# rubengooj/pl-svo

Measured on NVIDIA H100. Metric: frame-pair aligns/sec (VGA 5-lvl pyr, ~300pt+80ln), higher is better.
Workload: dtype f32 residuals, weights and chi2 (the reference's summation order, bit-exact); f64 per-pixel normal equations, solve and SE3

## Files before the change

### pl-svo_b200/csrc/align_kernel.cu

```cuda
#include <cuda_runtime.h>
#include <stdint.h>

#include "device_math.cuh"
#include "internal.h"

namespace plsvo {

namespace {

#ifdef PLSVO_PHASE_CLOCKS
enum {
  kPhSetup, kPhPtEval, kPhPtChi2, kPhSeg, kPhReduce,
  kPhSerRed, kPhSerSolve, kPhSerWalk, kPhSerSegSum, kPhSerBar1, kPhSerDecide, kPhSerFinal,
  kPhPair, kNumPhases
};
__device__ unsigned long long g_phase_clocks[kNumPhases];
#define PHASE_MARK(k)                        \
  do {                                       \
    const int ptid_ = fresh_tid();           \
    if ((ptid_ & 31) == 0) {                 \
      const long long now_ = clock64();      \
      ph_acc[ptid_ >> 5][k] += now_ - ph_t[ptid_ >> 5]; \
      ph_t[ptid_ >> 5] = now_;               \
    }                                        \
  } while (0)
#else
#define PHASE_MARK(k) \
  do {                \
  } while (0)
#endif

struct PairCtl {
  double R[9];
  double t[3];
  double model[7];
  double old_model[7];
  double T_ref[7];
  double ref_pos[3];
  double chi2_prev;
  double H_last[36];
  double scratch[36];
  double g[6];
  double x[6];
  unsigned long long mbar;
  long long n_meas_last;
  int pair;
  int flag;
  int stop;
  int iter;
  int n_seg_patches;
  int n_seg_slots;
  unsigned int patch_iters;
  unsigned int patch_levels;
  int iters_level[PLSVO_MAX_LEVELS];
  double cand[7];
  double candR[9];
  double cand_nm;
  double dscale, cJ, cJ2;
  float seg_chi2f;
  float chi2f;
  int n_opq;
  int chi2_flags;
};

struct Layout {
  uint32_t ctl, red, tot, chunk_tot, items, cnt, flat, opq, seg_N0, seg_N, seg_off, seg_slot, slot_seg, seg_term,
      seg_alive, pt_vis, xyz, tsc, img, total;
};

__host__ __device__ inline uint32_t align_up(uint32_t v, uint32_t a) { return (v + a - 1) / a * a; }

__host__ __device__ inline Layout make_layout(int n_pts, int n_segs, int max_patches, int max_seg_slots, int img_bytes,
                                              int nt) {
  Layout L;
  const uint32_t nw = (uint32_t)nt / 32u;
  const uint32_t rounds = ((uint32_t)n_pts + (uint32_t)nt - 1u) / (uint32_t)nt;
  const uint32_t n_chunks = ((uint32_t)n_pts + 31u) / 32u;
  uint32_t o = 0;
  L.ctl = o;
  o = align_up(o + (uint32_t)sizeof(PairCtl), 16);
  L.red = o;
  o += nw * 32u * 8u;
  L.tot = o;
  o += 32u * 8u;
  L.chunk_tot = o;
  o += 8u * (rounds * nw + 1u);
  L.items = o;
  o += 8u * 32u * (n_chunks + 1u);
  L.cnt = o;
  o += 4u * (n_chunks + 1u);
  L.flat = align_up(o, 8);
  o = L.flat + 8u * 64u;
  L.seg_N0 = o;
  o += 4u * (uint32_t)n_segs;
  L.seg_N = o;
  o += 4u * (uint32_t)n_segs;
  L.seg_off = o;
  o += 4u * (uint32_t)n_segs;
  L.seg_slot = o;
  o += 4u * (uint32_t)n_segs;
  L.slot_seg = o;
  o += 2u * (uint32_t)max_seg_slots;
  L.seg_term = align_up(o, 4);
  o = L.seg_term;
  o += 4u * (uint32_t)n_segs;
  L.seg_alive = o;
  o += (uint32_t)n_segs;
  L.pt_vis = o;
  o += (uint32_t)n_pts;
  L.xyz = align_up(o, 16);
  o = L.xyz + 3u * 8u * (uint32_t)max_patches;
  L.tsc = o;
  o += 16u * 4u * (uint32_t)nt;
  o = align_up(o, 128);
  L.img = o;
  o += (uint32_t)img_bytes + 16u;
  L.opq = align_up(o, 16);
  o = L.opq + 64u * (uint32_t)align_opq_cap(n_pts);
  L.total = o;
  return L;
}

__device__ __forceinline__ float bilin(float wTL, float wTR, float wBL, float wBR, float a, float b, float c, float d) {
  return __fadd_rn(__fadd_rn(__fadd_rn(__fmul_rn(wTL, a), __fmul_rn(wTR, b)), __fmul_rn(wBL, c)), __fmul_rn(wBR, d));
}

__device__ __forceinline__ bool patch_setup(double u, double v, int cols, int rows, int boundary, int& ui, int& vi,
                                            float& wTL, float& wTR, float& wBL, float& wBR) {
  const float uf = (float)u, vf = (float)v;
  const float fu = floorf(uf), fv = floorf(vf);
  ui = (int)fu;
  vi = (int)fv;
  if (ui < boundary || vi < boundary || ui >= cols - boundary || vi >= rows - boundary) return false;
  const float su = __fsub_rn(uf, fu), sv = __fsub_rn(vf, fv);
  const float omu = __fsub_rn(1.0f, su), omv = __fsub_rn(1.0f, sv);
  wTL = __fmul_rn(omu, omv);
  wTR = __fmul_rn(su, omv);
  wBL = __fmul_rn(omu, sv);
  wBR = __fmul_rn(su, sv);
  return true;
}

__device__ __noinline__ int seg_num_samples0(const double* spx, const double* epx, double length) {
  const double a0 = fabs(epx[0] - spx[0]), a1 = fabs(epx[1] - spx[1]);
  const double tan_dir = __ddiv_rn(fmin(a0, a1), fmax(a0, a1));
  const double sin_dir = __ddiv_rn(tan_dir, __dsqrt_rn(__dadd_rn(1.0, __dmul_rn(tan_dir, tan_dir))));
  const double correction = __dmul_rn(2.0, __dsqrt_rn(__dadd_rn(1.0, __dmul_rn(sin_dir, sin_dir))));
  double nd = __ddiv_rn(length, __dmul_rn(8.0, correction));
  if (!(nd >= 1.0)) nd = 1.0;
  if (nd > 1048576.0) nd = 1048576.0;
  return (int)(unsigned long long)nd;
}

__device__ __forceinline__ bool cam_in_frame(int ox, int oy, int boundary, int level, int width, int height) {
  return ox >= boundary && ox < width / (1 << level) - boundary && oy >= boundary &&
         oy < height / (1 << level) - boundary;
}

__device__ __forceinline__ void cam2world(const AlignArgs& a, const double* px, double* f) {
  const double x = __ddiv_rn(__dsub_rn(px[0], a.cx), a.fx), y = __ddiv_rn(__dsub_rn(px[1], a.cy), a.fy);
  const double n = __dsqrt_rn(__dadd_rn(__dadd_rn(__dmul_rn(x, x), __dmul_rn(y, y)), 1.0));
  f[0] = __ddiv_rn(x, n), f[1] = __ddiv_rn(y, n), f[2] = __ddiv_rn(1.0, n);
}

__device__ __forceinline__ void rank2_update(double* acc, double xn, double yn, double zi, double Sxx, double Sxy,
                                             double Syy, double Sxr, double Syr) {
  double r0[6], r1[6];
  const double xy = xn * yn;
  r0[0] = -zi, r0[1] = 0.0, r0[2] = xn * zi, r0[3] = xy, r0[4] = -(1.0 + xn * xn), r0[5] = yn;
  r1[0] = 0.0, r1[1] = -zi, r1[2] = yn * zi, r1[3] = 1.0 + yn * yn, r1[4] = -xy, r1[5] = -xn;
  double p[6], q[6];
#pragma unroll
  for (int i = 0; i < 6; ++i) {
    p[i] = Sxx * r0[i] + Sxy * r1[i];
    q[i] = Sxy * r0[i] + Syy * r1[i];
  }
  int idx = 0;
#pragma unroll
  for (int i = 0; i < 6; ++i)
#pragma unroll
    for (int j = i; j < 6; ++j) acc[idx++] += p[i] * r0[j] + q[i] * r1[j];
#pragma unroll
  for (int i = 0; i < 6; ++i) acc[21 + i] -= Sxr * r0[i] + Syr * r1[i];
}

__device__ __forceinline__ void load_row5(const uint8_t* row, int sh, uint32_t& lo, uint32_t& hi) {
  const uint32_t w0 = *reinterpret_cast<const uint32_t*>(row);
  const uint32_t w1 = *reinterpret_cast<const uint32_t*>(row + 4);
  lo = __funnelshift_r(w0, w1, sh);
  hi = w1 >> sh;
}
__device__ __forceinline__ float row_px(uint32_t lo, uint32_t hi, int k) {
  return k < 4 ? byte_to_float(lo, k) : byte_to_float(hi, 0);
}

__device__ __forceinline__ void project(const PairCtl* ctl, const AlignArgs& a, double xn, double yn, double zi, double& u,
                                        double& v) {
  const double* R = ctl->R;
  const double* t = ctl->t;
  const double xc = R[0] * xn + R[1] * yn + (R[2] + t[0] * zi);
  const double yc = R[3] * xn + R[4] * yn + (R[5] + t[1] * zi);
  const double zc = R[6] * xn + R[7] * yn + (R[8] + t[2] * zi);
  const double izc = __drcp_rn(zc);
  u = (a.fx * (xc * izc) + a.cx) * ctl->dscale;
  v = (a.fy * (yc * izc) + a.cy) * ctl->dscale;
}
__device__ __forceinline__ void load_row7(const uint8_t* row, int sh, float* g) {
  const uint32_t* wp = reinterpret_cast<const uint32_t*>(row);
  const uint32_t w0 = __ldg(wp), w1 = __ldg(wp + 1), w2 = __ldg(wp + 2);
  const uint32_t lo = __funnelshift_r(w0, w1, sh);
  const uint32_t hi = __funnelshift_r(w1, w2, sh);
  g[0] = byte_to_float(lo, 0);
  g[1] = byte_to_float(lo, 1);
  g[2] = byte_to_float(lo, 2);
  g[3] = byte_to_float(lo, 3);
  g[4] = byte_to_float(hi, 0);
  g[5] = byte_to_float(hi, 1);
  g[6] = byte_to_float(hi, 2);
}

template <bool weighted, int NT>
__device__ __forceinline__ bool eval_patch(const uint8_t* __restrict__ img, int pitch, int cols, int rows,
                                           const float4* __restrict__ cache, int MP, int p, double u, double v,
                                           double* S , float* __restrict__ tsc, float& tsum) {
  int ui, vi;
  float wTL, wTR, wBL, wBR;
  if (!patch_setup(u, v, cols, rows, 2, ui, vi, wTL, wTR, wBL, wBR)) return false;
  const int c0 = ui - 2;
  const int sh = (c0 & 3) * 8;
  const uint8_t* rowp = img + (size_t)(vi - 2) * pitch + (c0 & ~3);
  uint32_t ra_lo, ra_hi, rb_lo, rb_hi;
  load_row5(rowp, sh, ra_lo, ra_hi);
#ifdef PLSVO_FP32_SUMS
  float Sxx = 0.f, Sxy = 0.f, Syy = 0.f, Sxr = 0.f, Syr = 0.f;
#else
  double Sxx = 0, Sxy = 0, Syy = 0, Sxr = 0, Syr = 0;
#endif
  float acc_f = 0.f;
  const float4* cp = cache + p;
#pragma unroll 1
  for (int y = 0; y < 4; ++y) {
    rowp += pitch;
    load_row5(rowp, sh, rb_lo, rb_hi);
    const float4 ref4 = cp[0];
    const float4 dx4 = cp[4 * MP];
    const float4 dy4 = cp[8 * MP];
    cp += MP;
    const float refv[4] = {ref4.x, ref4.y, ref4.z, ref4.w};
    const float dxv[4] = {dx4.x, dx4.y, dx4.z, dx4.w};
    const float dyv[4] = {dy4.x, dy4.y, dy4.z, dy4.w};
#pragma unroll
    for (int x = 0; x < 4; ++x) {
      const float cur = bilin(wTL, wTR, wBL, wBR, row_px(ra_lo, ra_hi, x), row_px(ra_lo, ra_hi, x + 1),
                              row_px(rb_lo, rb_hi, x), row_px(rb_lo, rb_hi, x + 1));
      const float res = __fsub_rn(cur, refv[x]);
      const float dx = dxv[x], dy = dyv[x];
      const float ares = fabsf(res);
      const float nw = weighted ? -weight_rcp(ares) : -1.0f;
      const float nterm = weighted ? __fmul_rn(__fmul_rn(res, res), nw) : -ares;
      tsc[(y * 4 + x) * NT] = nterm;
      acc_f = __fsub_rn(acc_f, nterm);
#ifdef PLSVO_FP32_SUMS
      const float wdx = weighted ? __fmul_rn(-nw, dx) : dx, wdy = weighted ? __fmul_rn(-nw, dy) : dy;
      Sxx = fmaf(wdx, dx, Sxx);
      Sxy = fmaf(wdx, dy, Sxy);
      Syy = fmaf(wdy, dy, Syy);
      Sxr = fmaf(wdx, res, Sxr);
      Syr = fmaf(wdy, res, Syr);
#else
      const double dxd = (double)dx, dyd = (double)dy, rd = (double)res;
      const double nwdx = weighted ? (double)nw * dxd : -dxd;
      const double nwdy = weighted ? (double)nw * dyd : -dyd;
      Sxx = fma(-nwdx, dxd, Sxx);
      Sxy = fma(-nwdx, dyd, Sxy);
      Syy = fma(-nwdy, dyd, Syy);
      Sxr = fma(-nwdx, rd, Sxr);
      Syr = fma(-nwdy, rd, Syr);
#endif
    }
    ra_lo = rb_lo, ra_hi = rb_hi;
  }
  S[0] = (double)Sxx, S[1] = (double)Sxy, S[2] = (double)Syy, S[3] = (double)Sxr, S[4] = (double)Syr;
  tsum = acc_f;
  return true;
}

template <int NT>
__device__ __forceinline__ float chain16(float s, const float* tsc) {
#pragma unroll
  for (int k = 0; k < 16; ++k) s = __fsub_rn(s, tsc[k * NT]);
  return s;
}
template <int NT>
__device__ __forceinline__ void chain16x2(float& s0, float& s1, const float* tsc) {
#pragma unroll
  for (int k = 0; k < 16; ++k) {
    const float t = tsc[k * NT];
    s0 = __fsub_rn(s0, t);
    s1 = __fsub_rn(s1, t);
  }
}

__device__ __forceinline__ void precompute_patch(const uint8_t* __restrict__ img, int pitch, int ui, int vi, float wTL,
                                                 float wTR, float wBL, float wBR, float4* __restrict__ cache, int MP,
                                                 int p) {
  const int c0 = ui - 3;
  const int sh = (c0 & 3) * 8;
  const uint8_t* rowp = img + (size_t)(vi - 3) * pitch + (c0 & ~3);
  float g0[7], g1[7], Va[6], Vb[6], Vc[6];
  load_row7(rowp, sh, g0);
  load_row7(rowp + pitch, sh, g1);
#pragma unroll
  for (int c = 0; c < 6; ++c) Va[c] = bilin(wTL, wTR, wBL, wBR, g0[c], g0[c + 1], g1[c], g1[c + 1]);
  rowp += 2 * pitch;
  load_row7(rowp, sh, g0);
#pragma unroll
  for (int c = 0; c < 6; ++c) Vb[c] = bilin(wTL, wTR, wBL, wBR, g1[c], g1[c + 1], g0[c], g0[c + 1]);
  float4* cp = cache + p;
#pragma unroll 1
  for (int y = 0; y < 4; ++y) {
    rowp += pitch;
    load_row7(rowp, sh, g1);
#pragma unroll
    for (int c = 0; c < 6; ++c) Vc[c] = bilin(wTL, wTR, wBL, wBR, g0[c], g0[c + 1], g1[c], g1[c + 1]);
    float refv[4], dxv[4], dyv[4];
#pragma unroll
    for (int x = 0; x < 4; ++x) {
      refv[x] = Vb[x + 1];
      dxv[x] = __fmul_rn(0.5f, __fsub_rn(Vb[x + 2], Vb[x]));
      dyv[x] = __fmul_rn(0.5f, __fsub_rn(Vc[x + 1], Va[x + 1]));
    }
    cp[0] = make_float4(refv[0], refv[1], refv[2], refv[3]);
    cp[4 * MP] = make_float4(dxv[0], dxv[1], dxv[2], dxv[3]);
    cp[8 * MP] = make_float4(dyv[0], dyv[1], dyv[2], dyv[3]);
    cp += MP;
#pragma unroll
    for (int c = 0; c < 6; ++c) Va[c] = Vb[c], Vb[c] = Vc[c];
#pragma unroll
    for (int c = 0; c < 7; ++c) g0[c] = g1[c];
  }
}

__device__ __forceinline__ void zero_gradients(float4* cache, int MP, int p) {
  const float4 z = make_float4(0.f, 0.f, 0.f, 0.f);
#pragma unroll
  for (int y = 0; y < 8; ++y) cache[(4 + y) * MP + p] = z;
}

__device__ __noinline__ void gn_solve(PairCtl* ctl, const double* tot, int level) {
  ctl->n_meas_last = (long long)tot[28];
  ctl->patch_iters += (unsigned int)tot[29];
  ctl->iters_level[level] += 1;
  double xx[6];
  {
    double Hu[21], gg[6];
#pragma unroll
    for (int i = 0; i < 21; ++i) Hu[i] = tot[i];
#pragma unroll
    for (int i = 0; i < 6; ++i) gg[i] = tot[21 + i];
    if (!ldlt6_reg(Hu, gg, xx)) {
      double* H = ctl->H_last;
      int idx = 0;
      for (int i = 0; i < 6; ++i)
        for (int j = i; j < 6; ++j) {
          H[i * 6 + j] = tot[idx];
          H[j * 6 + i] = tot[idx];
          ++idx;
        }
      for (int i = 0; i < 6; ++i) ctl->g[i] = tot[21 + i];
      ldlt6_solve(H, ctl->g, ctl->x, ctl->scratch);
#pragma unroll
      for (int i = 0; i < 6; ++i) xx[i] = ctl->x[i];
    }
  }
  if (isnan(xx[0])) ctl->stop = 1;
  double mx[6];
  double nm = 0.0;
#pragma unroll
  for (int i = 0; i < 6; ++i) {
    mx[i] = -xx[i];
    nm = fmax(nm, fabs(xx[i]));
  }
  SE3q model;
  model.q.x = ctl->model[0], model.q.y = ctl->model[1], model.q.z = ctl->model[2], model.q.w = ctl->model[3];
  model.t = v3(ctl->model[4], ctl->model[5], ctl->model[6]);
  const SE3q cand = se3_mul(model, se3_exp(mx));
  se3_store(cand, ctl->cand);
  quat_to_R(cand.q, ctl->candR);
  ctl->cand_nm = nm;
}

__device__ __noinline__ void gn_decide(PairCtl* ctl, const double* tot, float chi2f, int n_iter, double eps) {
  const double new_chi2 = (double)(chi2f / (float)(unsigned long long)ctl->n_meas_last);
  const bool reject = (ctl->iter > 0 && new_chi2 > ctl->chi2_prev) || ctl->stop;
  int flag;
  if (reject) {
    for (int i = 0; i < 7; ++i) ctl->model[i] = ctl->old_model[i];
    Quat q;
    q.x = ctl->model[0], q.y = ctl->model[1], q.z = ctl->model[2], q.w = ctl->model[3];
    quat_to_R(q, ctl->R);
    flag = 1;
  } else {
    for (int i = 0; i < 7; ++i) ctl->old_model[i] = ctl->model[i], ctl->model[i] = ctl->cand[i];
    for (int i = 0; i < 9; ++i) ctl->R[i] = ctl->candR[i];
    ctl->chi2_prev = new_chi2;
    flag = (ctl->cand_nm <= eps) ? 1 : 0;
  }
  ctl->t[0] = ctl->model[4], ctl->t[1] = ctl->model[5], ctl->t[2] = ctl->model[6];
  ctl->iter += 1;
  if (ctl->iter >= n_iter) flag = 1;
  if (flag) {
    int idx = 0;
    for (int i = 0; i < 6; ++i)
      for (int j = i; j < 6; ++j) {
        ctl->H_last[i * 6 + j] = tot[idx];
        ctl->H_last[j * 6 + i] = tot[idx];
        ++idx;
      }
  }
  ctl->flag = flag;
}

__device__ __forceinline__ int fresh_tid() {
  int t;
  asm volatile("mov.u32 %0, %%tid.x;" : "=r"(t));
  return t;
}

__device__ __forceinline__ void named_barrier_sync(int id, int nthreads) {
  asm volatile("bar.sync %0, %1;" ::"r"(id), "r"(nthreads) : "memory");
}
__device__ __forceinline__ void named_barrier_arrive(int id, int nthreads) {
  asm volatile("bar.arrive %0, %1;" ::"r"(id), "r"(nthreads) : "memory");
}

__device__ __forceinline__ uint2 make_item(uint32_t Ae, uint32_t Ao, uint32_t ef, uint32_t opaque, uint32_t slot) {
  uint2 it;
  it.x = Ae | slot;
  it.y = ((Ao - Ae) & 0xffffu) | (ef << 16) | (opaque << 24);
  return it;
}

template <int NT, int MINB>
__global__ void __launch_bounds__(NT, MINB) sparse_img_align_kernel(const AlignArgs a) {
  constexpr int NW = NT / 32;
  constexpr int WALK = NW > 1 ? 1 : 0;
  constexpr int SEGW = NW > 2 ? 2 : WALK;
  constexpr int kSerialThreads = 32 * (NW > 2 ? 3 : (NW > 1 ? 2 : 1));
  extern __shared__ __align__(128) unsigned char smem[];
  const int tid = threadIdx.x, lane = tid & 31, warp = tid >> 5;
  const int MP = a.max_patches;
  const Layout L = make_layout(a.n_pts, a.n_segs, MP, a.max_seg_slots, a.smem_img_bytes, NT);
  PairCtl* ctl = reinterpret_cast<PairCtl*>(smem + L.ctl);
  double* red = reinterpret_cast<double*>(smem + L.red);
  double* tot = reinterpret_cast<double*>(smem + L.tot);
  double* chunk_tot = reinterpret_cast<double*>(smem + L.chunk_tot);
  uint2* items = reinterpret_cast<uint2*>(smem + L.items);
  int* item_cnt = reinterpret_cast<int*>(smem + L.cnt);
  float* opq = reinterpret_cast<float*>(smem + L.opq);
  uint8_t* seg_alive = smem + L.seg_alive;
  int* seg_N0 = reinterpret_cast<int*>(smem + L.seg_N0);
  int* seg_N = reinterpret_cast<int*>(smem + L.seg_N);
  int* seg_off = reinterpret_cast<int*>(smem + L.seg_off);
  int* seg_slot = reinterpret_cast<int*>(smem + L.seg_slot);
  uint16_t* slot_seg = reinterpret_cast<uint16_t*>(smem + L.slot_seg);
  const int max_slots = a.max_seg_slots;
  float* seg_term = reinterpret_cast<float*>(smem + L.seg_term);
  uint8_t* pt_vis = smem + L.pt_vis;
  uint8_t* img_s = smem + L.img;
  float4* cache = a.ws_cache + (size_t)blockIdx.x * kCacheRows * MP;
  double* xyz = reinterpret_cast<double*>(smem + L.xyz);
  float* tsc = reinterpret_cast<float*>(smem + L.tsc) + tid;
  uint2* flat = reinterpret_cast<uint2*>(smem + L.flat);
  double* seg_px = a.ws_segpx + (size_t)blockIdx.x * 2 * a.max_seg_patches;
  const int RS = a.rec_cap * NT;
  double* rec = a.ws_rec + (size_t)blockIdx.x * 5 * RS;
  uint64_t* bar = reinterpret_cast<uint64_t*>(&ctl->mbar);
  if (tid == 0) {
    mbar_init(bar, 1);
    fence_mbarrier_init();
    fence_proxy_async();
  }
  __syncthreads();
  uint32_t bar_parity = 0;
#ifdef PLSVO_PHASE_CLOCKS
  __shared__ unsigned long long ph_acc[NW][kNumPhases];
  __shared__ long long ph_t[NW];
  if (lane == 0) {
    for (int k = 0; k < kNumPhases; ++k) ph_acc[warp][k] = 0ull;
    ph_t[warp] = clock64();
  }
#endif

  for (;;) {
    __syncthreads();
    if (tid == 0) {
      const int nb = (int)atomicAdd(a.work_counter, 1u);
      if (a.gate_chunk > 0 && nb < a.B) {
        const unsigned need = (unsigned)(nb / a.gate_chunk) + 1u;
        while (*reinterpret_cast<const volatile unsigned int*>(a.arrived) < need) __nanosleep(1000);
        __threadfence_system();
      }
      ctl->pair = nb;
    }
    __syncthreads();
    const int b = ctl->pair;
    if (b >= a.B) break;

    const int np = min(max(a.pt_count ? a.pt_count[b] : a.n_pts, 0), a.n_pts);
    const int ns = min(max(a.seg_count ? a.seg_count[b] : a.n_segs, 0), a.n_segs);
    const size_t po = (size_t)b * a.n_pts, so = (size_t)b * a.n_segs;

    if (np == 0 && ns == 0) {
      if (tid == 0) {
        for (int i = 0; i < 7; ++i) a.out_T[(size_t)b * 7 + i] = a.T_cur_w[(size_t)b * 7 + i];
        a.out_n_tracked[b] = 0;
        for (int i = 0; i < 36; ++i) a.out_H[(size_t)b * 36 + i] = 0.0;
        for (int l = 0; l < PLSVO_MAX_LEVELS; ++l) a.out_iters[(size_t)b * PLSVO_MAX_LEVELS + l] = 0;
        a.out_status[b] = 1;
        a.out_patch_iters[b] = 0;
        a.out_patch_levels[b] = 0;
      }
      for (int j = tid; j < a.n_segs; j += NT) a.out_seg_killed[so + j] = 0;
      continue;
    }

    if (tid == 0) {
      const SE3q T_ref = se3_load(a.T_ref_w + (size_t)b * 7);
      const SE3q T_cur = se3_load(a.T_cur_w + (size_t)b * 7);
      const SE3q T_ref_inv = se3_inverse(T_ref);
      const SE3q model = se3_mul(T_cur, T_ref_inv);
      se3_store(T_ref, ctl->T_ref);
      se3_store(model, ctl->model);
      ctl->ref_pos[0] = T_ref_inv.t.x, ctl->ref_pos[1] = T_ref_inv.t.y, ctl->ref_pos[2] = T_ref_inv.t.z;
      quat_to_R(model.q, ctl->R);
      ctl->t[0] = model.t.x, ctl->t[1] = model.t.y, ctl->t[2] = model.t.z;
      ctl->chi2_prev = 1e10;
      ctl->stop = 0;
      ctl->n_meas_last = 0;
      ctl->patch_iters = 0;
      ctl->patch_levels = 0;
      ctl->chi2_flags = 0;
      ctl->n_opq = 0;
      for (int i = 0; i < 36; ++i) ctl->H_last[i] = 0.0;
      for (int l = 0; l < PLSVO_MAX_LEVELS; ++l) ctl->iters_level[l] = 0;
    }
    if (a.derive_from >= 0) {
      for (int l = a.derive_from + 1; l <= a.max_level; ++l) {
        const int cols = a.width >> l, rows = a.height >> l;
        const int pin = (int)a.pitch[l - 1], pout = (int)a.pitch[l];
#pragma unroll 1
        for (int which = 0; which < 2; ++which) {
          const uint8_t* src = (which ? a.cur_img[l - 1] : a.ref_img[l - 1]) + (size_t)b * a.stride[l - 1];
          uint8_t* dst = const_cast<uint8_t*>(which ? a.cur_img[l] : a.ref_img[l]) + (size_t)b * a.stride[l];
          for (int y = warp; y < rows; y += NW) {
            const uint8_t* r0 = src + (size_t)(2 * y) * pin;
            for (int x = lane; x < cols; x += 32)
              dst[(size_t)y * pout + x] = (uint8_t)(((int)r0[2 * x] + (int)r0[2 * x + 1] + (int)r0[pin + 2 * x] + (int)r0[pin + 2 * x + 1]) >> 2);
          }
        }
        __syncthreads();
      }
      asm volatile("fence.proxy.async;" ::: "memory");
      __syncthreads();
    }
    __syncthreads();
    const double rpx = ctl->ref_pos[0], rpy = ctl->ref_pos[1], rpz = ctl->ref_pos[2];

    for (int i = tid; i < np; i += NT) {
      pt_vis[i] = 0;
      double fd[3];
      const double* f = fd;
      if (a.pt_f) f = a.pt_f + (po + i) * 3;
      else cam2world(a, a.pt_px + (po + i) * 2, fd);
      double depth;
      if (a.pt_depth) {
        depth = a.pt_depth[po + i];
      } else {
        const double* pos = a.pt_pos + (po + i) * 3;
        const double dx = pos[0] - rpx, dy = pos[1] - rpy, dz = pos[2] - rpz;
        depth = sqrt(dx * dx + dy * dy + dz * dz);
      }
      const double zi = 1.0 / (f[2] * depth);
      xyz[3 * i + 0] = (f[0] * depth) * zi;
      xyz[3 * i + 1] = (f[1] * depth) * zi;
      xyz[3 * i + 2] = zi;
    }
    for (int j = tid; j < ns; j += NT) {
      seg_alive[j] = a.seg_valid ? (a.seg_valid[so + j] ? 1 : 0) : 1;
      seg_N0[j] = seg_num_samples0(a.seg_spx + (so + j) * 2, a.seg_epx + (so + j) * 2, a.seg_length[so + j]);
    }
    unsigned int my_patch_levels = 0;
    const int n_chunks = (np + 31) >> 5;
    const int rounds = (np + NT - 1) / NT;

    for (int level = a.max_level; level >= a.min_level; --level) {
      PHASE_MARK(kPhPair);
      const int cols = a.width >> level, rows = a.height >> level;
      const int pitch = (int)a.pitch[level];
      const float scale = 1.0f / (float)(1 << level);
      const double dscale = (double)scale;
      const uint8_t* ref_img = a.ref_img[level] + (size_t)b * a.stride[level];
      const uint8_t* cur_img_g = a.cur_img[level] + (size_t)b * a.stride[level];
      const bool stage = a.img_in_smem[level] != 0;
      const uint8_t* cur_img = stage ? img_s : cur_img_g;
      __syncthreads();
      if (tid == 0) {
        if (stage) {
          const uint32_t bytes = (uint32_t)rows * (uint32_t)pitch;
          fence_proxy_async();
          mbar_expect_tx(bar, bytes);
          bulk_g2s(img_s, cur_img_g, bytes, bar);
        }
        ctl->iter = 0;
        for (int i = 0; i < 7; ++i) ctl->old_model[i] = ctl->model[i];
        ctl->dscale = dscale;
        ctl->cJ = fabs(a.fx) / (double)(1 << level);
        ctl->cJ2 = ctl->cJ * ctl->cJ;
      }
      for (int j = tid; j < ns; j += NT) {
        int N = 0;
        if (seg_alive[j]) {
          const double* spx = a.seg_spx + (so + j) * 2;
          const double* epx = a.seg_epx + (so + j) * 2;
          const int sx = (int)(spx[0] * dscale), sy = (int)(spx[1] * dscale);
          const int ex = (int)(epx[0] * dscale), ey = (int)(epx[1] * dscale);
          if (cam_in_frame(sx, sy, 3, level, a.width, a.height) && cam_in_frame(ex, ey, 3, level, a.width, a.height))
            N = 1 + ((seg_N0[j] - 1) >> level);
        }
        seg_N[j] = N;
        seg_term[j] = 0.f;
      }
      for (int q = tid; q < max_slots; q += NT) slot_seg[q] = 0xffffu;
      __syncthreads();
      if (warp == 0) {
        int carry = 0;
        for (int base = 0; base < ns; base += 32) {
          const int j = base + lane;
          const int v = (j < ns) ? seg_N[j] : 0;
          int incl = v;
#pragma unroll
          for (int d = 1; d < 32; d <<= 1) {
            const int n = __shfl_up_sync(0xffffffffu, incl, d);
            if (lane >= d) incl += n;
          }
          if (j < ns) seg_off[j] = carry + incl - v;
          carry += __shfl_sync(0xffffffffu, incl, 31);
        }
        int slot_base = 0;
        for (int cls = 5; cls >= 0; --cls) {
          int cnt = 0;
          for (int base = 0; base < ns; base += 32) {
            const int j = base + lane;
            const int N = (j < ns) ? seg_N[j] : 0;
            int k = -1;
            if (N > 0) {
              k = 0;
              while ((1 << k) < N && k < 5) ++k;
            }
            const unsigned m = __ballot_sync(0xffffffffu, k == cls);
            if (k == cls) seg_slot[j] = slot_base + ((cnt + __popc(m & ((1u << lane) - 1u))) << cls);
            cnt += __popc(m);
          }
          slot_base += cnt << cls;
        }
        if (lane == 0) {
          ctl->n_seg_patches = carry;
          ctl->n_seg_slots = slot_base;
        }
      }
      __syncthreads();
      const int n_sp = min(ctl->n_seg_patches, a.max_seg_patches);
      const int n_patches = np + n_sp;
      const int n_seg_slots = min((ctl->n_seg_slots + 31) & ~31, max_slots);
      for (int j = tid; j < ns; j += NT) {
        const int N = seg_N[j];
        if (N == 0) continue;
        const double* spx = a.seg_spx + (so + j) * 2;
        const double* epx = a.seg_epx + (so + j) * 2;
        const double dif[2] = {epx[0] - spx[0], epx[1] - spx[1]};
        const double nm1 = (double)(unsigned long long)(N - 1);
        const double inc2d0 = dif[0] * dscale / nm1, inc2d1 = dif[1] * dscale / nm1;
        double px0 = spx[0] * dscale, px1 = spx[1] * dscale;
        double sfd[3], efd[3];
        const double *sf = sfd, *ef = efd;
        if (a.seg_sf) sf = a.seg_sf + (so + j) * 3;
        else cam2world(a, spx, sfd);
        if (a.seg_ef) ef = a.seg_ef + (so + j) * 3;
        else cam2world(a, epx, efd);
        double p_depth, q_depth;
        if (a.seg_sdepth) {
          p_depth = a.seg_sdepth[so + j];
        } else {
          const double* sp = a.seg_spos + (so + j) * 3;
          const double d0 = sp[0] - rpx, d1 = sp[1] - rpy, d2 = sp[2] - rpz;
          p_depth = sqrt(d0 * d0 + d1 * d1 + d2 * d2);
        }
        if (a.seg_edepth) {
          q_depth = a.seg_edepth[so + j];
        } else {
          const double* ep = a.seg_epos + (so + j) * 3;
          const double d0 = ep[0] - rpx, d1 = ep[1] - rpy, d2 = ep[2] - rpz;
          q_depth = sqrt(d0 * d0 + d1 * d1 + d2 * d2);
        }
        const double P0 = sf[0] * p_depth, P1 = sf[1] * p_depth, P2 = sf[2] * p_depth;
        const double Q0 = ef[0] * q_depth, Q1 = ef[1] * q_depth, Q2 = ef[2] * q_depth;
        const double i0 = (Q0 - P0) / nm1, i1 = (Q1 - P1) / nm1, i2 = (Q2 - P2) / nm1;
        double X = P0, Y = P1, Z = P2;
        const int off = seg_off[j];
        {
          int g = 1;
          while (g < N && g < 32) g <<= 1;
          const int s0 = seg_slot[j];
          for (int n = 0; n < g; ++n)
            if (s0 + n < max_slots) slot_seg[s0 + n] = (uint16_t)j;
        }
        for (int n = 0; n < N; ++n) {
          const int sp_idx = off + n;
          if (sp_idx < n_sp) {
            seg_px[2 * sp_idx] = px0;
            seg_px[2 * sp_idx + 1] = px1;
            const double zi = 1.0 / Z;
            xyz[3 * (np + sp_idx) + 0] = X * zi;
            xyz[3 * (np + sp_idx) + 1] = Y * zi;
            xyz[3 * (np + sp_idx) + 2] = zi;
          }
          px0 += inc2d0, px1 += inc2d1;
          X += i0, Y += i1, Z += i2;
        }
      }
      __syncthreads();
      for (int p = tid; p < n_patches; p += NT) {
        double u, v;
        const bool is_pt = p < np;
        if (is_pt) {
          if (a.pt_valid && !a.pt_valid[po + p]) continue;
          const double* px = a.pt_px + (po + p) * 2;
          u = px[0] * dscale, v = px[1] * dscale;
        } else {
          u = seg_px[2 * (p - np)], v = seg_px[2 * (p - np) + 1];
        }
        int ui, vi;
        float wTL, wTR, wBL, wBR;
        const bool in = patch_setup(u, v, cols, rows, 3, ui, vi, wTL, wTR, wBL, wBR);
        if (!in) {
          if (!is_pt || pt_vis[p]) zero_gradients(cache, MP, p);
          continue;
        }
        if (is_pt) pt_vis[p] = 1;
        precompute_patch(ref_img, pitch, ui, vi, wTL, wTR, wBL, wBR, cache, MP, p);
        ++my_patch_levels;
      }
      if (stage) {
        mbar_wait(bar, bar_parity);
        bar_parity ^= 1u;
      }
      __syncthreads();
      PHASE_MARK(kPhSetup);

      for (;;) {
        int n_pt_acc = 0;
#ifdef PLSVO_TREE_CHI2
        double chi2_tree = 0.0;
#endif
        double acc[27];
#pragma unroll
        for (int i = 0; i < 27; ++i) acc[i] = 0.0;
        double prefix_rounds = 0.0;
        for (int r = 0; r < rounds; ++r) {
          const int c = r * NW + warp;
          const int p = c * 32 + lane;
          float Tf = 0.f;
          bool ok = false;
          if (p < np && pt_vis[p]) {
            const double* X = xyz + 3 * p;
            double u, v;
            project(ctl, a, X[0], X[1], X[2], u, v);
            double S[5];
            ok = eval_patch<true, NT>(cur_img, pitch, cols, rows, cache, MP, p, u, v, S, tsc, Tf);
            if (ok) {
              const double cJ = ctl->cJ, cJ2 = ctl->cJ2;
              rank2_update(acc, X[0], X[1], X[2], S[0] * cJ2, S[1] * cJ2, S[2] * cJ2, S[3] * cJ, S[4] * cJ);
              n_pt_acc += 1;
            }
          }
          if (!ok) Tf = 0.f;
          PHASE_MARK(kPhPtEval);
#ifdef PLSVO_TREE_CHI2
          chi2_tree += (double)Tf;
#else
          if (c >= n_chunks) {
            named_barrier_arrive(2, NT);
            PHASE_MARK(kPhPtChi2);
            continue;
          }
          double incl = (double)Tf;
#pragma unroll
          for (int d = 1; d < 32; d <<= 1) {
            const double n = __shfl_up_sync(0xffffffffu, incl, d);
            if (lane >= d) incl += n;
          }
          if (lane == 31) chunk_tot[c] = incl;
          named_barrier_sync(2, NT);
          double P = prefix_rounds;
#pragma unroll
          for (int w = 0; w < NW; ++w) {
            const double tw = (r * NW + w < n_chunks) ? chunk_tot[r * NW + w] : 0.0;
            if (w < warp) P += tw;
            prefix_rounds += tw;
          }
          P += incl - (double)Tf;
          if (c < n_chunks) {
            const double delta = (double)(16 * (p + 2)) * 6.0e-8 + 2.0e-6;
            const double lo = P * (1.0 - delta), hi = (P + (double)Tf) * (1.0 + delta);
            const int e_lo = (__double2hiint(lo) >> 20) - 1023, e_hi = (__double2hiint(hi) >> 20) - 1023;
            uint32_t ef = 0, opaque = 0, Ae = 0, Ao = 0, slot = 0;
            if (Tf == 0.f) {
              if (P != 0.0 && e_lo == e_hi && e_lo >= -100 && e_lo <= 100) ef = (uint32_t)(e_lo + 127);
              else if (P != 0.0) ef = 255u;
            } else if (P == 0.0) {
              opaque = 1u;
            } else if (e_lo != e_hi || e_lo < -100 || e_lo > 100) {
              opaque = 1u;
            } else {
              ef = (uint32_t)(e_lo + 127);
              const uint32_t b0 = ef << 23;
              float s0 = __uint_as_float(b0), s1 = __uint_as_float(b0 | 1u);
              chain16x2<NT>(s0, s1, tsc);
              Ae = __float_as_uint(s0) - b0;
              Ao = __float_as_uint(s1) - (b0 | 1u);
            }
            if (opaque) {
              const int idx = atomicAdd(&ctl->n_opq, 1);
              if (idx < align_opq_cap(a.n_pts)) {
                slot = (uint32_t)idx;
#pragma unroll
                for (int k = 0; k < 16; ++k) opq[idx * 16 + k] = tsc[k * NT];
              } else {
                atomicOr(&ctl->chi2_flags, 1);
                opaque = 0u;
              }
            }
            const uint32_t ef_prev = __shfl_up_sync(0xffffffffu, ef, 1);
            const uint32_t op_prev = __shfl_up_sync(0xffffffffu, opaque, 1);
            uint32_t head = (lane == 0 || opaque || op_prev || ef != ef_prev) ? 1u : 0u;
            const uint32_t heads = __ballot_sync(0xffffffffu, head);
#pragma unroll
            for (int d = 1; d < 32; d <<= 1) {
              const uint32_t pAe = __shfl_up_sync(0xffffffffu, Ae, d);
              const uint32_t pAo = __shfl_up_sync(0xffffffffu, Ao, d);
              const uint32_t phead = __shfl_up_sync(0xffffffffu, head, d);
              if (lane >= d && !head) {
                const uint32_t nAe = pAe + ((pAe & 1u) ? Ao : Ae);
                const uint32_t nAo = pAo + ((pAo & 1u) ? Ae : Ao);
                Ae = nAe, Ao = nAo;
                head = phead;
              }
            }
            const bool tail = lane == 31 || ((heads >> (lane + 1)) & 1u);
            const uint32_t tails = __ballot_sync(0xffffffffu, tail);
            if (tail) items[c * 32 + __popc(tails & ((1u << lane) - 1u))] = make_item(Ae, Ao, ef, opaque, slot);
            if (lane == 0) item_cnt[c] = __popc(tails);
          }
#endif
          PHASE_MARK(kPhPtChi2);
        }
        int n_meas_acc = 16 * n_pt_acc, n_patch_acc = n_pt_acc;
        for (int base = (NW - 1 - warp) * 32; base < n_seg_slots; base += NT) {
          const int q = base + lane;
          const int j = slot_seg[q];
          const bool has = j < ns;
          const bool seg_ok = has && seg_alive[j];
          const int Ns = has ? seg_N[j] : 0;
          const int N = seg_ok ? Ns : 0;
          const int off = has ? seg_off[j] : 0;
          const int n0 = has ? q - seg_slot[j] : 0;
          int G = 1;
          while (G < Ns && G < 32) G <<= 1;
          const int gbase = lane - n0;
          int trips = seg_ok ? (Ns + G - 1) / G : 0, gmax = seg_ok ? G : 0;
#pragma unroll
          for (int d = 16; d >= 1; d >>= 1) {
            trips = max(trips, __shfl_xor_sync(0xffffffffu, trips, d));
            gmax = max(gmax, __shfl_xor_sync(0xffffffffu, gmax, d));
          }
          float s_tok = 0.f;
          int first_bad = 0x7fffffff;
          unsigned ok_trips = 0u;
          double S[5] = {0.0, 0.0, 0.0, 0.0, 0.0};
          int p = 0;
          for (int trip = 0; trip < trips; ++trip) {
            const int n = n0 + trip * G;
            const bool active = n < N;
            float Tf = 0.f;
            bool ok = false;
            if (active) {
              p = np + off + n;
              double u, v;
              project(ctl, a, xyz[3 * p + 0], xyz[3 * p + 1], xyz[3 * p + 2], u, v);
              ok = eval_patch<false, NT>(cur_img, pitch, cols, rows, cache, MP, p, u, v, S, tsc, Tf);
              if (ok) {
                ok_trips |= 1u << (trip & 31);
                if (trips > 1) {
                  if (trip < a.rec_cap) {
                    double* rp = rec + trip * NT + tid;
#pragma unroll
                    for (int k = 0; k < 5; ++k) rp[k * RS] = S[k];
                  } else {
                    atomicOr(&ctl->chi2_flags, 4);
                  }
                }
              } else {
                first_bad = min(first_bad, n);
              }
            }
            for (int g = 0; g < gmax; ++g) {
              const float prev = __shfl_sync(0xffffffffu, s_tok, gbase + ((n0 - 1) & (G - 1)));
              if (n0 == g) {
                const float s_in = (g == 0 && trip == 0) ? 0.f : prev;
                s_tok = (active && ok) ? (s_in == 0.f ? Tf : chain16<NT>(s_in, tsc)) : s_in;
              }
            }
          }
          float res_ = __shfl_sync(0xffffffffu, s_tok, gbase + G - 1);
#pragma unroll
          for (int d = 16; d >= 1; d >>= 1) {
            const int fb = __shfl_xor_sync(0xffffffffu, first_bad, d);
            if (d < G) first_bad = min(first_bad, fb);
          }
          double sH = 0.0, sJ = 0.0;
          if (N > 0 && n0 == 0) {
            const bool good = first_bad >= N;
            n_patch_acc += good ? N : first_bad;
            res_ = (float)((double)res_ / (double)(unsigned long long)N);
            if (good && (double)res_ < 200.0) {
              const float w = (float)(1.0 / (1.0 + (double)res_));
              sH = (double)w / (double)res_ * ctl->cJ2;
              sJ = (double)w * ctl->cJ;
              seg_term[j] = __fmul_rn(__fmul_rn(res_, res_), w);
#ifdef PLSVO_TREE_CHI2
              chi2_tree += (double)seg_term[j];
#endif
              n_meas_acc += 1;
            } else {
              seg_term[j] = 0.f;
              seg_alive[j] = 0;
            }
          }
          sH = __shfl_sync(0xffffffffu, sH, gbase);
          sJ = __shfl_sync(0xffffffffu, sJ, gbase);
          if (sH != 0.0 || sJ != 0.0) {
            if (trips == 1) {
              if (ok_trips) rank2_update(acc, xyz[3 * p + 0], xyz[3 * p + 1], xyz[3 * p + 2], S[0] * sH, S[1] * sH, S[2] * sH,
                                         S[3] * sJ, S[4] * sJ);
            } else {
              for (int trip = 0; trip < trips && trip < a.rec_cap; ++trip) {
                if (!((ok_trips >> (trip & 31)) & 1u)) continue;
                const int pp = np + off + n0 + trip * G;
                const double* rp = rec + trip * NT + tid;
                rank2_update(acc, xyz[3 * pp + 0], xyz[3 * pp + 1], xyz[3 * pp + 2], rp[0] * sH, rp[RS] * sH, rp[2 * RS] * sH,
                             rp[3 * RS] * sJ, rp[4 * RS] * sJ);
              }
            }
          }
        }
        PHASE_MARK(kPhSeg);
        double v[32];
#pragma unroll
        for (int i = 0; i < 27; ++i) v[i] = acc[i];
#ifdef PLSVO_TREE_CHI2
        v[27] = chi2_tree;
#else
        v[27] = 0.0;
#endif
        v[28] = (double)n_meas_acc;
        v[29] = (double)n_patch_acc;
        v[30] = 0.0, v[31] = 0.0;
        const double mine = warp_reduce32(v, lane);
        red[fresh_tid()] = mine;
        __syncthreads();
        PHASE_MARK(kPhReduce);
        if (warp == 0) {
          double s = 0.0;
#pragma unroll
          for (int w = 0; w < NW; ++w) s += red[w * 32 + lane];
          tot[lane] = s;
          __syncwarp();
          PHASE_MARK(kPhSerRed);
          if (lane == 0) gn_solve(ctl, tot, level);
          PHASE_MARK(kPhSerSolve);
        }
#ifdef PLSVO_TREE_CHI2
        if (warp == WALK && lane == 0) ctl->chi2f = 0.f;
        if (false) {
#else
        if ((fresh_tid() >> 5) == WALK) {
#endif
          float s = 0.f;
          uint32_t bad = 0;
          for (int c = 0; c < n_chunks;) {
            const int cc = c + lane;
            const int my_cnt = (cc < n_chunks) ? item_cnt[cc] : 0;
            int incl = my_cnt;
#pragma unroll
            for (int d = 1; d < 32; d <<= 1) {
              const int n = __shfl_up_sync(0xffffffffu, incl, d);
              if (lane >= d) incl += n;
            }
            const int nfit = max(1, __popc(__ballot_sync(0xffffffffu, cc < n_chunks && incl <= 64)));
            for (int j = 0; j < nfit; ++j) {
              const int cnt_j = __shfl_sync(0xffffffffu, my_cnt, j), off_j = __shfl_sync(0xffffffffu, incl - my_cnt, j);
              if (lane < cnt_j) flat[off_j + lane] = items[(c + j) * 32 + lane];
            }
            const int total = __shfl_sync(0xffffffffu, incl, nfit - 1);
            __syncwarp();
            for (int b0 = 0; b0 < total; b0 += 32) {
              uint2 it = make_uint2(0u, 0u);
              if (b0 + lane < total) it = flat[b0 + lane];
              float4 q0 = make_float4(0.f, 0.f, 0.f, 0.f), q1 = q0, q2 = q0, q3 = q0;
              if ((it.y >> 24) & 1u) {
                const float4* o4 = reinterpret_cast<const float4*>(opq + it.x * 16);
                q0 = o4[0], q1 = o4[1], q2 = o4[2], q3 = o4[3];
              }
              const float tr[16] = {q0.x, q0.y, q0.z, q0.w, q1.x, q1.y, q1.z, q1.w, q2.x, q2.y, q2.z, q2.w, q3.x, q3.y, q3.z, q3.w};
              const int m = min(32, total - b0);
              for (int k = 0; k < m; ++k) {
                const uint32_t ix = __shfl_sync(0xffffffffu, it.x, k), iy = __shfl_sync(0xffffffffu, it.y, k);
                if ((iy >> 24) & 1u) {
                  float so = s;
#pragma unroll
                  for (int i = 0; i < 16; ++i) so = __fsub_rn(so, tr[i]);
                  s = __shfl_sync(0xffffffffu, so, k);
                } else {
                  const uint32_t dA = (uint32_t)(int)(short)(iy & 0xffffu);
                  if (ix | dA) {
                    uint32_t bits = __float_as_uint(s);
                    bad |= (bits >> 23) ^ ((iy >> 16) & 0xffu);
                    bits += (bits & 1u) ? ix + dA : ix;
                    s = __uint_as_float(bits);
                  }
                }
              }
            }
            __syncwarp();
            c += nfit;
          }
          if (lane == 0) {
            if (ctl->n_opq > align_opq_cap(a.n_pts)) {
              double e = 0.0;
              for (int c = 0; c < n_chunks; ++c) e += chunk_tot[c];
              s = (float)e;
            }
            if (bad) atomicOr(&ctl->chi2_flags, 2);
            ctl->chi2f = s;
            ctl->n_opq = 0;
          }
          PHASE_MARK(kPhSerWalk);
        }
        if ((fresh_tid() >> 5) == SEGW) {
          float s2 = 0.f;
#pragma unroll 8
          for (int j = 0; j < ns; ++j) s2 = __fadd_rn(s2, seg_term[j]);
          if (lane == 0) ctl->seg_chi2f = s2;
          PHASE_MARK(kPhSerSegSum);
        }
        const int stid = fresh_tid();
        if (NW > 1 && (stid & ~31) < kSerialThreads) {
          named_barrier_sync(1, kSerialThreads);
          PHASE_MARK(kPhSerBar1);
        }
#ifdef PLSVO_TREE_CHI2
        if (stid == 0) gn_decide(ctl, tot, (float)tot[27], a.n_iter, a.eps);
#else
        if (stid == 0) gn_decide(ctl, tot, __fadd_rn(ctl->chi2f, ctl->seg_chi2f), a.n_iter, a.eps);
#endif
        PHASE_MARK(kPhSerDecide);
        __syncthreads();
        PHASE_MARK(kPhSerFinal);
        if (ctl->flag) break;
      }
    }

    {
      unsigned int v = my_patch_levels;
#pragma unroll
      for (int d = 16; d >= 1; d >>= 1) v += __shfl_xor_sync(0xffffffffu, v, d);
      if (lane == 0 && v) atomicAdd(&ctl->patch_levels, v);
    }
    for (int j = tid; j < a.n_segs; j += NT) {
      const bool valid0 = (j < ns) && (a.seg_valid ? a.seg_valid[so + j] != 0 : true);
      a.out_seg_killed[so + j] = (valid0 && !seg_alive[j]) ? 1 : 0;
    }
    __syncthreads();
    if (tid == 0) {
      SE3q model, T_ref;
      model.q.x = ctl->model[0], model.q.y = ctl->model[1], model.q.z = ctl->model[2], model.q.w = ctl->model[3];
      model.t = v3(ctl->model[4], ctl->model[5], ctl->model[6]);
      T_ref.q.x = ctl->T_ref[0], T_ref.q.y = ctl->T_ref[1], T_ref.q.z = ctl->T_ref[2], T_ref.q.w = ctl->T_ref[3];
      T_ref.t = v3(ctl->T_ref[4], ctl->T_ref[5], ctl->T_ref[6]);
      const SE3q T_cur = se3_mul(model, T_ref);
      se3_store(T_cur, a.out_T + (size_t)b * 7);
      a.out_n_tracked[b] = ctl->n_meas_last / 16;
      for (int i = 0; i < 36; ++i) a.out_H[(size_t)b * 36 + i] = ctl->H_last[i];
      for (int l = 0; l < PLSVO_MAX_LEVELS; ++l) a.out_iters[(size_t)b * PLSVO_MAX_LEVELS + l] = ctl->iters_level[l];
      a.out_status[b] = (ctl->stop ? 2 : 0) | (ctl->chi2_flags << 2);
      a.out_patch_iters[b] = ctl->patch_iters;
      a.out_patch_levels[b] = ctl->patch_levels;
    }
  }
#ifdef PLSVO_PHASE_CLOCKS
  PHASE_MARK(kPhPair);
  if (lane == 0)
    for (int k = 0; k < kNumPhases; ++k) atomicAdd(&g_phase_clocks[k], ph_acc[warp][k]);
#endif
}

}

namespace {
__global__ void weight_selftest_kernel(uint32_t n, uint32_t seed, unsigned long long* mismatch) {
  unsigned long long bad = 0;
  for (uint32_t i = blockIdx.x * blockDim.x + threadIdx.x; i < n; i += gridDim.x * blockDim.x) {
    uint32_t h = (i ^ seed) * 2654435761u;
    h ^= h >> 15;
    h *= 2246822519u;
    h ^= h >> 13;
    float a;
    if (i & 1) {
      a = __uint_as_float(h % 0x43800000u);
    } else {
      a = (float)(h & 0xffffff) * (1.0f / 65536.0f);
    }
    const float fast = weight_rcp(a);
    const float ref = (float)(1.0 / (1.0 + (double)a));
    if (__float_as_uint(fast) != __float_as_uint(ref)) ++bad;
  }
  if (bad) atomicAdd(mismatch, bad);
}
}

cudaError_t weight_selftest_launch(uint32_t n, uint32_t seed, unsigned long long* d_mismatch, cudaStream_t s) {
  weight_selftest_kernel<<<528, 256, 0, s>>>(n, seed, d_mismatch);
  return cudaGetLastError();
}

size_t align_smem_bytes(int n_pts, int n_segs, int max_patches, int max_seg_slots, int img_bytes, int threads) {
  return make_layout(n_pts, n_segs, max_patches, max_seg_slots, img_bytes, threads).total;
}

#define PLSVO_ALIGN_VARIANTS(X) X(64, 8) X(96, 7) X(96, 5) X(128, 5) X(128, 4) X(160, 3) X(192, 2) X(256, 2)

namespace {
template <int NT, int MINB>
cudaError_t prepare_t(size_t smem_bytes, int* ctas_per_sm) {
  cudaError_t e = cudaFuncSetAttribute(sparse_img_align_kernel<NT, MINB>, cudaFuncAttributeMaxDynamicSharedMemorySize,
                                       (int)smem_bytes);
  if (e != cudaSuccess) return e;
  e = cudaFuncSetAttribute(sparse_img_align_kernel<NT, MINB>, cudaFuncAttributePreferredSharedMemoryCarveout,
                           cudaSharedmemCarveoutMaxShared);
  if (e != cudaSuccess) return e;
  return cudaOccupancyMaxActiveBlocksPerMultiprocessor(ctas_per_sm, sparse_img_align_kernel<NT, MINB>, NT, smem_bytes);
}
}

cudaError_t align_kernel_prepare(int threads, int min_blocks, size_t smem_bytes, int* ctas_per_sm) {
#define X(NT, MB) \
  if (threads == NT && min_blocks == MB) return prepare_t<NT, MB>(smem_bytes, ctas_per_sm);
  PLSVO_ALIGN_VARIANTS(X)
#undef X
  return cudaErrorInvalidValue;
}

cudaError_t align_kernel_launch(const AlignArgs& a, int grid, int threads, int min_blocks, size_t smem_bytes,
                                cudaStream_t s) {
#define X(NT, MB)                                                            \
  if (threads == NT && min_blocks == MB) {                                   \
    sparse_img_align_kernel<NT, MB><<<grid, NT, smem_bytes, s>>>(a);         \
    return cudaGetLastError();                                               \
  }
  PLSVO_ALIGN_VARIANTS(X)
#undef X
  return cudaErrorInvalidValue;
}

}

#ifdef PLSVO_PHASE_CLOCKS
extern "C" int plsvo_phase_clocks(unsigned long long* out, int reset) {
  cudaError_t e = cudaDeviceSynchronize();
  if (e == cudaSuccess) e = cudaMemcpyFromSymbol(out, plsvo::g_phase_clocks, sizeof(plsvo::g_phase_clocks));
  if (e == cudaSuccess && reset) {
    const unsigned long long zero[plsvo::kNumPhases] = {};
    e = cudaMemcpyToSymbol(plsvo::g_phase_clocks, zero, sizeof(zero));
  }
  return (int)e;
}
#endif
```

Baseline: 782,100.

## Parallelize chi2 bit-walk with warp scan and warp-wide GN decision

Replaces the serial per-item shuffle walk of the bit-exact chi2 accumulation with a segmented warp prefix scan over the (even, odd) increment pairs. Only runs separated by opaque items are applied serially, and the exponent check is recomputed per lane. gn_decide is spread across a full warp, with lanes writing model, R and H_last entries in parallel. Other serial threads now arrive at the named barrier instead of syncing on it. This cuts serial-path latency per GN iteration but adds shuffle-heavy scan work and new risk to bit-exact correctness.

```diff
diff --git a/pl-svo_b200/csrc/align_kernel.cu b/pl-svo_b200/csrc/align_kernel.cu
--- a/pl-svo_b200/csrc/align_kernel.cu
+++ b/pl-svo_b200/csrc/align_kernel.cu
@@ -390,35 +390,47 @@
   ctl->cand_nm = nm;
 }
 
-__device__ __noinline__ void gn_decide(PairCtl* ctl, const double* tot, float chi2f, int n_iter, double eps) {
+__device__ __noinline__ void gn_decide(PairCtl* ctl, const double* tot, float chi2f, int n_iter, double eps, int lane) {
   const double new_chi2 = (double)(chi2f / (float)(unsigned long long)ctl->n_meas_last);
-  const bool reject = (ctl->iter > 0 && new_chi2 > ctl->chi2_prev) || ctl->stop;
-  int flag;
+  const int iter = ctl->iter + 1;
+  const bool reject = (iter > 1 && new_chi2 > ctl->chi2_prev) || ctl->stop;
+  const int flag = (reject || ctl->cand_nm <= eps || iter >= n_iter) ? 1 : 0;
+  double m = 0.0, r = 0.0, h0 = 0.0, h1 = 0.0;
+  if (lane < 7) m = reject ? ctl->old_model[lane] : ctl->cand[lane];
+  const double m_old = (lane < 7) ? ctl->model[lane] : 0.0;
+  if (lane < 9 && !reject) r = ctl->candR[lane];
+  if (flag) {
+    int i = lane / 6, j = lane % 6;
+    int lo = min(i, j), hi = max(i, j);
+    h0 = tot[lo * 6 - lo * (lo - 1) / 2 + hi - lo];
+    i = (lane + 32) / 6, j = (lane + 32) % 6;
+    lo = min(i, j), hi = max(i, j);
+    if (lane < 4) h1 = tot[lo * 6 - lo * (lo - 1) / 2 + hi - lo];
+  }
+  __syncwarp();
+  if (lane < 7) {
+    ctl->model[lane] = m;
+    if (!reject) ctl->old_model[lane] = m_old;
+    if (lane >= 4) ctl->t[lane - 4] = m;
+  }
   if (reject) {
-    for (int i = 0; i < 7; ++i) ctl->model[i] = ctl->old_model[i];
-    Quat q;
-    q.x = ctl->model[0], q.y = ctl->model[1], q.z = ctl->model[2], q.w = ctl->model[3];
-    quat_to_R(q, ctl->R);
-    flag = 1;
-  } else {
-    for (int i = 0; i < 7; ++i) ctl->old_model[i] = ctl->model[i], ctl->model[i] = ctl->cand[i];
-    for (int i = 0; i < 9; ++i) ctl->R[i] = ctl->candR[i];
-    ctl->chi2_prev = new_chi2;
-    flag = (ctl->cand_nm <= eps) ? 1 : 0;
-  }
-  ctl->t[0] = ctl->model[4], ctl->t[1] = ctl->model[5], ctl->t[2] = ctl->model[6];
-  ctl->iter += 1;
-  if (ctl->iter >= n_iter) flag = 1;
+    if (lane == 0) {
+      Quat q;
+      q.x = m, q.y = ctl->old_model[1], q.z = ctl->old_model[2], q.w = ctl->old_model[3];
+      quat_to_R(q, ctl->R);
+    }
+  } else if (lane < 9) {
+    ctl->R[lane] = r;
+  }
   if (flag) {
-    int idx = 0;
-    for (int i = 0; i < 6; ++i)
-      for (int j = i; j < 6; ++j) {
-        ctl->H_last[i * 6 + j] = tot[idx];
-        ctl->H_last[j * 6 + i] = tot[idx];
-        ++idx;
-      }
-  }
-  ctl->flag = flag;
+    ctl->H_last[lane] = h0;
+    if (lane < 4) ctl->H_last[lane + 32] = h1;
+  }
+  if (lane == 0) {
+    if (!reject) ctl->chi2_prev = new_chi2;
+    ctl->iter = iter;
+    ctl->flag = flag;
+  }
 }
 
 __device__ __forceinline__ int fresh_tid() {
@@ -1023,28 +1035,53 @@
                 q0 = o4[0], q1 = o4[1], q2 = o4[2], q3 = o4[3];
               }
               const float tr[16] = {q0.x, q0.y, q0.z, q0.w, q1.x, q1.y, q1.z, q1.w, q2.x, q2.y, q2.z, q2.w, q3.x, q3.y, q3.z, q3.w};
-              const int m = min(32, total - b0);
-              for (int k = 0; k < m; ++k) {
-                const uint32_t ix = __shfl_sync(0xffffffffu, it.x, k), iy = __shfl_sync(0xffffffffu, it.y, k);
-                if ((iy >> 24) & 1u) {
+              const bool opaque = (it.y >> 24) & 1u;
+              const uint32_t dA = (uint32_t)(int)(short)(it.y & 0xffffu);
+              const uint32_t Ae = opaque ? 0u : it.x, Ao = opaque ? 0u : it.x + dA;
+              const uint32_t opm = __ballot_sync(0xffffffffu, opaque);
+              const uint32_t heads = (opm << 1) | 1u;
+              uint32_t iAe = Ae, iAo = Ao, head = (heads >> lane) & 1u;
+#pragma unroll
+              for (int d = 1; d < 32; d <<= 1) {
+                const uint32_t pAe = __shfl_up_sync(0xffffffffu, iAe, d);
+                const uint32_t pAo = __shfl_up_sync(0xffffffffu, iAo, d);
+                const uint32_t phead = __shfl_up_sync(0xffffffffu, head, d);
+                if (lane >= d && !head) {
+                  const uint32_t nAe = pAe + ((pAe & 1u) ? iAo : iAe);
+                  const uint32_t nAo = pAo + ((pAo & 1u) ? iAe : iAo);
+                  iAe = nAe, iAo = nAo;
+                  head = phead;
+                }
+              }
+              uint32_t run_in = 0u;
+              uint32_t rest = opm;
+              for (int h = 0; h < 32;) {
+                const int k = rest ? __ffs(rest) - 1 : 31;
+                uint32_t bits = __float_as_uint(s);
+                if (lane >= h && lane <= k) run_in = bits;
+                const uint32_t cAe = __shfl_sync(0xffffffffu, iAe, k), cAo = __shfl_sync(0xffffffffu, iAo, k);
+                bits += (bits & 1u) ? cAo : cAe;
+                s = __uint_as_float(bits);
+                if (rest) {
                   float so = s;
 #pragma unroll
                   for (int i = 0; i < 16; ++i) so = __fsub_rn(so, tr[i]);
                   s = __shfl_sync(0xffffffffu, so, k);
-                } else {
-                  const uint32_t dA = (uint32_t)(int)(short)(iy & 0xffffu);
-                  if (ix | dA) {
-                    uint32_t bits = __float_as_uint(s);
-                    bad |= (bits >> 23) ^ ((iy >> 16) & 0xffu);
-                    bits += (bits & 1u) ? ix + dA : ix;
-                    s = __uint_as_float(bits);
-                  }
+                  rest &= rest - 1u;
                 }
+                h = k + 1;
+              }
+              const uint32_t xAe = __shfl_up_sync(0xffffffffu, iAe, 1), xAo = __shfl_up_sync(0xffffffffu, iAo, 1);
+              if (!opaque && (it.x | dA)) {
+                const bool first = (heads >> lane) & 1u;
+                const uint32_t entry = run_in + (first ? 0u : ((run_in & 1u) ? xAo : xAe));
+                bad |= (entry >> 23) ^ ((it.y >> 16) & 0xffu);
               }
             }
             __syncwarp();
             c += nfit;
           }
+          bad = __any_sync(0xffffffffu, bad != 0u);
           if (lane == 0) {
             if (ctl->n_opq > align_opq_cap(a.n_pts)) {
               double e = 0.0;
@@ -1065,15 +1102,18 @@
           PHASE_MARK(kPhSerSegSum);
         }
         const int stid = fresh_tid();
-        if (NW > 1 && (stid & ~31) < kSerialThreads) {
+        if (stid < 32) {
           named_barrier_sync(1, kSerialThreads);
           PHASE_MARK(kPhSerBar1);
-        }
 #ifdef PLSVO_TREE_CHI2
-        if (stid == 0) gn_decide(ctl, tot, (float)tot[27], a.n_iter, a.eps);
+          gn_decide(ctl, tot, (float)tot[27], a.n_iter, a.eps, stid);
 #else
-        if (stid == 0) gn_decide(ctl, tot, __fadd_rn(ctl->chi2f, ctl->seg_chi2f), a.n_iter, a.eps);
+          gn_decide(ctl, tot, __fadd_rn(ctl->chi2f, ctl->seg_chi2f), a.n_iter, a.eps, stid);
 #endif
+        } else if (stid < kSerialThreads) {
+          named_barrier_arrive(1, kSerialThreads);
+          PHASE_MARK(kPhSerBar1);
+        }
         PHASE_MARK(kPhSerDecide);
         __syncthreads();
         PHASE_MARK(kPhSerFinal);
```

New measurement: 793,100, median of 6. About the same (+1.4%).
